# apache/yunikorn-k8shim

Measured on AMD Instinct MI355X. Metric: pod×node predicate evals/sec + decisions/sec, 50k nodes × 1M pods, higher is better.
Workload: dtype int64; 1 GPU; configs[2]: 50k nodes x 1M pods, NodeResourcesFit + TaintToleration + NodeAffinity; nodes_per_gpu=50000, total_nodes=50000, pods=1000000, templates=2000, pod_classes=2061, signature_planes=327, unique_requests=False, spread=False, gang_size=0, parallelism=single GPU

## Files before the change

yunikorn-k8shim_amd/csrc/engine/engine.hip:

```cpp
#include "../../../include/ykpred.h"

#include <hip/hip_runtime.h>
#include <dlfcn.h>
#include <rccl/rccl.h>

#include <algorithm>
#include <chrono>
#include <cstdio>
#include <cstdlib>
#include <cstring>
#include <mutex>
#include <string>
#include <unordered_map>
#include <vector>

#include "kernels.hip.h"

using ykk::i64;
using ykk::u64;

namespace {

thread_local std::string g_create_error;

// ... 187 lines not shown
  int64_t spread_cells = 0;
  bool spread_dirty = true;
  int res_vectors = 0;
  std::vector<i64> h_dim_val;
  std::vector<int32_t> h_dim_of;
  std::vector<int32_t> h_stage_rows;
  DevBuf d_dim_val, d_dim_order, d_dim_chunk_dim, d_dim_chunk_begin, d_dim_chunk_len, d_res_rows;
  int dim_chunks = 0;
  int walk_rows = 256;
  int wave_combine_below = 16;
  int n_big = 0, walk_chunks = 0, index_rows = 0;
  int NCB = 0;
  DevBuf d_big_dim, d_walk_big, d_walk_begin, d_walk_len, d_sfree_c, d_pmask_c, d_sfree_r, d_pmask_r, d_rbits_c;
  std::vector<int32_t> h_res_rows;
  std::vector<int32_t> h_row_pos;
  std::vector<int32_t> h_row_big;
  std::vector<int32_t> h_sorted_off;
  DevBuf d_sorted, d_sorted_off, d_ent_c;
  int sweep_min_run = 1;
  int sweep_groups = 0;
  bool sweep_ready = false;
  std::vector<int32_t> h_class_sweep;
  int sweep_rows[ykk::kMaxIdxRows] = {0, 0}, sweep_row_off[ykk::kMaxIdxRows + 1] = {0, 0, 0}, sweep_runs = 0;
  int index_rows_needed = 0;
  DevBuf d_agree;
  DevBuf d_explain;
  DevBuf d_headroom;
  DevBuf d_bytes_gather;
  DevBuf d_topo_agree;
  u64 dict_digest = 0;
  int fuse_rows = 1;
  int fuse_wpl = 0;
  int fuse_count = 0, fuse_row_count = 0;
  bool fuse_ready = false;
  DevBuf d_fuse_rec;
  int fuse_combos = 0;
  int fuse_combine = 1;
  DevBuf d_fuse_combo_rec, d_fuse_combo;
  std::vector<uint8_t> h_class_fused;
  int run_decide = 1;
  int run_ranges = 0, n_decide_list = 0, run_decide_classes = -1;
  bool win_partial = false;
  DevBuf d_run_ranges, d_no_decide, d_glin_r;
  int class_runs = 1;
  int class_runs_min_rows = 16;
  int run_classes = 0, run_units = 0, run_rows = 0;
  DevBuf d_run_classes, d_run_units;
  DevBuf d_sweep_rows, d_sweep_runs, d_sweep_units;
  int sweep_units[ykk::kMaxIdxRows] = {0, 0}, sweep_unit_off[ykk::kMaxIdxRows + 1] = {0, 0, 0};
  DevBuf d_chunk_list_b0;
  int NCB0 = 0;
  DevBuf d_walk2_order, d_walk2_big, d_walk2_begin, d_walk2_len;
  int walk2_chunks = -1;
  DevBuf d_first_r;
  static constexpr bool decide_skip = true;
  DevBuf d_chunk_list_b;
  DevBuf d_slice_general;
  DevBuf d_slice_desc;
  DevBuf d_pfx_r;
  DevBuf d_idx_c;
  DevBuf d_win_r;
  int idx_stride = 0;
  DevBuf d_sig_tol, d_sig_tolflags, d_sig_ports, d_swanted;
  DevBuf d_sig_aff_flags, d_sig_aff_off, d_sig_aff_terms, d_sig_pre_off, d_sig_pre_terms;
  bool specs_set = false;

  int P = 0, C = 0, NC = 0;
  std::vector<int32_t> h_pod_spec, h_pod_pin;
  DevBuf d_pod_spec, d_pod_pin, d_pod_class;
  DevBuf d_class_sig, d_class_pin, d_class_first, d_class_word, d_chunk_class, d_chunk_begin, d_chunk_len, d_chunk_first, d_members;
  std::unordered_map<ClassKey, int32_t, ClassKeyHash> class_ids;
  std::vector<int32_t> h_pod_class, h_pod_slot;
  std::vector<int32_t> h_pod_row;
  int rows_total = 0, rows_a = 0, row_capacity = 0;
  DevBuf d_pod_row;
  bool bands_enabled = true;
  int band_steps = 0;
  int band_steps_now = 128;
  int round_batched = -1;
  int round_node_assume = 1;
  int round_prof = 0;
  int fail_after = 0;
  int sig_wpl = 0;
  int combine_slices = 1;
  int decide_groups_from = 16384;
  int early_counts = 1;
  int max_lds_bytes = 64 * 1024;
  int num_cus = 256;
  int n_bands = 0, n_band_steps = 0, n_classes_a = 0, n_fix_rows = 0;
  std::vector<int32_t> h_class_slot_a;
  DevBuf d_band_tab, d_class_rows_a, d_class_list_a, d_class_slot_a, d_fix_row, d_fix_slot, d_chunk_zone;
  DevBuf d_class_list_b;
  int n_classes_b = 0;
  std::vector<int32_t> h_ch_zone;
  std::vector<uint8_t> h_row_stale;
  std::vector<int32_t> h_class_sig, h_class_pin, h_class_first, h_class_live;
  std::vector<std::vector<int32_t>> h_class_chunks;
  std::vector<int32_t> h_members, h_ch_class, h_ch_begin, h_ch_len, h_ch_first;
  int patch_chunks = 0;
  bool rank_valid = false;
  uint64_t specs_version = 1, ranked_specs_version = 0, ranked_nodes_epoch = 0;
  unsigned ranked_pre = 0, ranked_filt = 0;
  bool ranked_has_first = false;
  DevBuf d_round;
  DevBuf d_fx_off, d_fx_cls, d_fx_cnt, d_fx_occ, d_sp_sig_of;
  uint64_t fx_version = 0;
  bool fx_contrib = false, fx_ports = false;
  std::vector<int32_t> h_fx_off;
  std::vector<int32_t> h_fx_cls;
  std::vector<uint8_t> h_fx_occupies;
  DevBuf d_patches, d_rows, d_row_count, d_row_best;
  unsigned last_pre = 0, last_filt = 0;
  bool last_eval_valid = false;
  DevBuf d_class_count, d_class_best;
  bool pods_set = false, classes_dirty = true;
  int chunk_members = ykk::kChunkMembers;
  bool chunk_sorted = true;
  int combine_lds_bytes = 40000;

  DevBuf d_bitmap, d_counts, d_decisions, d_keys, d_scratch;
  void* last_bitmap = nullptr;
  int64_t last_bitmap_rows = 0;
  void *last_counts = nullptr, *last_decisions = nullptr, *last_keys = nullptr;

  hipStream_t aux_stream = nullptr;
  hipEvent_t ev_fork = nullptr, ev_planes = nullptr, ev_join = nullptr, ev_counts = nullptr, ev_zero = nullptr;
  hipStream_t peek_stream = nullptr;
  hipEvent_t ev_eval_done = nullptr;
  void* peek_pinned = nullptr;
  size_t peek_pinned_bytes = 0;

  struct GraphKey {
    uint64_t version;
    unsigned pre, filt, options;
    void *bitmap, *counts, *decisions, *keys;
    bool operator==(const GraphKey& o) const {
      return version == o.version && pre == o.pre && filt == o.filt && options == o.options && bitmap == o.bitmap && counts == o.counts &&
             decisions == o.decisions && keys == o.keys;
    }
  };
  std::vector<std::pair<GraphKey, hipGraphExec_t>> graphs;
  std::vector<GraphKey> seen;
  uint64_t tables_version = 1;
  bool graph_disabled = true;

  ncclComm_t comm = nullptr;
  int comm_rank = 0, comm_world = 1, node_offset = 0;
  int64_t round_exchanges = 0;
  void* h_round_pinned = nullptr;
  size_t h_round_pinned_bytes = 0;
  int64_t rounds_batched = 0, round_batched_asks = 0, round_batches = 0, rounds_sequential = 0, round_sequential_asks = 0;
  int forced_stride = 0;
  DevBuf d_gathered, d_gathered_map, d_xkey, d_xcand;
  bool last_has_keys = false;
  DevBuf d_class_rows_all, d_gathered_classes, d_class_rows_slot, d_class_sig_ident, d_expand_count, d_layout_hash, d_gathered_pod_class, d_row_pod;
  int ident_classes = 0;
  uint64_t layout_version = 1, layout_hashed_version = 0, layout_hash_value = 0, row_pod_version = 0;
  uint64_t ask_epoch = 1, hdr_epoch = 0;
  std::vector<uint64_t> hdr_cache;
  uint64_t nodes_epoch = 1, hist_epoch = 0;
  uint64_t bitmap_epoch = 0;

  int64_t n_full_evals = 0, n_node_patches = 0, n_row_patches = 0, n_queries = 0, n_gathers = 0, n_uploads = 0;

  hipEvent_t ev[2 * YKPRED_MAX_TIMED_KERNELS + 2]{};
  bool ev_ready = false;
// ... 1059 lines not shown

#define YK_SERIALISE(eng) \
  std::unique_lock<std::recursive_mutex> engine_lock; \
  if (eng) engine_lock = std::unique_lock<std::recursive_mutex>((eng)->mu)

extern "C" {

int32_t ykpred_abi_version(void) { return YKPRED_ABI_VERSION; }

const char* ykpred_last_error(const ykpred_engine_t* e) { return e ? e->err.c_str() : g_create_error.c_str(); }

int32_t ykpred_create(const ykpred_config_t* cfg, ykpred_engine_t** out) {
  if (!cfg || !out) {
    g_create_error = "null argument";
    return YKPRED_E_INVALID;
  }
  if (cfg->abi_version != YKPRED_ABI_VERSION) {
    g_create_error = "ABI version mismatch";
    return YKPRED_E_INVALID;
  }
  if (cfg->num_resources < 3 || cfg->num_resources > ykk::kMaxR || cfg->taint_words < 1 || cfg->taint_words > ykk::kMaxKT ||
      cfg->label_words < 1 || cfg->label_words > ykk::kMaxWTotal) {
    g_create_error = "config out of range: need 3<=R<=8, 1<=KT<=4, 1<=W<=32";
    return YKPRED_E_UNSUPPORTED;
  }
  if (cfg->topology_keys < 0 || cfg->topology_keys > ykk::kMaxKD || cfg->selector_classes < 0 || cfg->selector_classes > 4096 ||
      cfg->port_words < 0 || cfg->port_words > ykk::kMaxKP) {
    g_create_error = "config out of range: need 0<=KD<=8 topology keys, 0<=KS<=4096 selector classes, 0<=KP<=4 port words";
    return YKPRED_E_UNSUPPORTED;
  }
  int ndev = 0;
  hipError_t s = hipGetDeviceCount(&ndev);
  if (s != hipSuccess || ndev <= 0) {
    g_create_error = std::string("no HIP device: ") + hipGetErrorString(s) + " (libykpred has no CPU fallback)";
    return YKPRED_E_DEVICE;
  }
  if (cfg->device < 0 || cfg->device >= ndev) {
    g_create_error = "device ordinal out of range";
    return YKPRED_E_INVALID;
  }
  s = hipSetDevice(cfg->device);
  if (s != hipSuccess) {
    g_create_error = std::string("hipSetDevice: ") + hipGetErrorString(s);
    return YKPRED_E_DEVICE;
  }
  auto* e = new ykpred_engine();
  e->cfg = *cfg;
  e->R = cfg->num_resources;
  e->KT = cfg->taint_words;
  e->W = cfg->label_words;
  e->KD = cfg->topology_keys;
  e->KS = cfg->selector_classes;
  e->KP = cfg->port_words;
  if (cfg->reserved[0] >= 1 && cfg->reserved[0] <= ykk::kChunkMembers) e->chunk_members = cfg->reserved[0];
  e->chunk_sorted = cfg->reserved[1] != 1;
  if (cfg->reserved[2] > 0 && cfg->reserved[2] <= 160 * 1024) e->combine_lds_bytes = cfg->reserved[2];
  if (cfg->reserved[2] < 0) e->combine_lds_bytes = 0;
  if (cfg->reserved[4] > 0) e->walk_rows = cfg->reserved[4];
  if (cfg->reserved[5] > 0) e->wave_combine_below = cfg->reserved[5];
  if (cfg->reserved[5] < 0) e->wave_combine_below = 0;
  if (cfg->reserved[6] < 0) e->bands_enabled = false;
  if (cfg->reserved[6] > 0) e->band_steps = std::min(256, std::max(4, (cfg->reserved[6] + 3) / 4 * 4));
  e->graph_disabled = cfg->reserved[3] != 1;
  {
    int lds = 0;
    if (hipDeviceGetAttribute(&lds, hipDeviceAttributeMaxSharedMemoryPerBlock, cfg->device) == hipSuccess && lds > 0) e->max_lds_bytes = lds;
    int cus = 0;
    if (hipDeviceGetAttribute(&cus, hipDeviceAttributeMultiprocessorCount, cfg->device) == hipSuccess && cus > 0) e->num_cus = cus;
  }
  if (const char* tune = getenv("YKPRED_TUNE")) {
    std::string text(tune);
    size_t at = 0;
    while (at < text.size()) {
      size_t stop = text.find(',', at);
      if (stop == std::string::npos) stop = text.size();
      const std::string item = text.substr(at, stop - at);
      at = stop + 1;
      if (item.empty()) continue;
      const size_t eq = item.find('=');
      const std::string key = item.substr(0, eq);
      const int val = eq == std::string::npos ? 1 : atoi(item.c_str() + eq + 1);
      if (key == "walk_rows") e->walk_rows = std::max(val, 1);
      else if (key == "sig_wpl") e->sig_wpl = val;
      else if (key == "combine_slices") e->combine_slices = val;
      else if (key == "decide_groups_from") e->decide_groups_from = val;
      else if (key == "graph") e->graph_disabled = val != 1;
      else if (key == "early_counts") e->early_counts = val;
      else if (key == "band_steps") {
        e->bands_enabled = val >= 0;
        e->band_steps = val > 0 ? std::min(256, std::max(4, (val + 3) / 4 * 4)) : 0;
      } else if (key == "chunk_members") e->chunk_members = std::min(std::max(val, 1), (int)ykk::kChunkMembers);
      else if (key == "wave_combine_below") e->wave_combine_below = std::max(val, 0);
      else if (key == "fail_after") e->fail_after = std::max(val, 0);
      else if (key == "round_prof") e->round_prof = val;
      else if (key == "round_batched") e->round_batched = val;
      else if (key == "round_node_assume") e->round_node_assume = val;
      else if (key == "sweep_min_run") e->sweep_min_run = std::max(val, 0);
      else if (key == "sweep_groups") e->sweep_groups = std::max(val, 0);
      else if (key == "class_runs") e->class_runs = val;
      else if (key == "run_decide") e->run_decide = val;
      else if (key == "fuse_rows") e->fuse_rows = val;
      else if (key == "fuse_wpl") e->fuse_wpl = val;
      else if (key == "fuse_combine") e->fuse_combine = val;
      else if (key == "class_runs_min_rows") e->class_runs_min_rows = std::max(val, 1);
      else {
        g_create_error = "YKPRED_TUNE: unknown key '" + key + "'";
        delete e;
        return YKPRED_E_INVALID;
      }
    }
  }
  s = hipStreamCreateWithFlags(&e->own_stream, hipStreamNonBlocking);
  if (s != hipSuccess) {
    g_create_error = std::string("hipStreamCreate: ") + hipGetErrorString(s);
    delete e;
    return YKPRED_E_DEVICE;
  }
  {
    int lo = 0, hi = 0;
    (void)hipDeviceGetStreamPriorityRange(&lo, &hi);
    if (hipStreamCreateWithPriority(&e->aux_stream, hipStreamNonBlocking, hi) != hipSuccess)
      (void)hipStreamCreateWithFlags(&e->aux_stream, hipStreamNonBlocking);
  }
  if (hipStreamCreateWithFlags(&e->peek_stream, hipStreamNonBlocking) != hipSuccess) e->peek_stream = nullptr;
  (void)hipEventCreateWithFlags(&e->ev_eval_done, hipEventDisableTiming);
  (void)hipEventCreateWithFlags(&e->ev_fork, hipEventDisableTiming);
  (void)hipEventCreateWithFlags(&e->ev_join, hipEventDisableTiming);
  (void)hipEventCreateWithFlags(&e->ev_planes, hipEventDisableTiming);
  (void)hipEventCreateWithFlags(&e->ev_counts, hipEventDisableTiming);
  (void)hipEventCreateWithFlags(&e->ev_zero, hipEventDisableTiming);
  for (auto& ev : e->ev) (void)hipEventCreate(&ev);
  e->ev_ready = true;
  *out = e;
  return YKPRED_OK;
}

void ykpred_destroy(ykpred_engine_t* e) {
  if (!e) return;
  (void)hipSetDevice(e->cfg.device);
  (void)hipDeviceSynchronize();
  if (e->comm) (void)rccl()->CommDestroy(e->comm);
  e->comm = nullptr;
  for (DevBuf* b : {&e->d_gathered, &e->d_gathered_map, &e->d_xkey, &e->d_xcand}) b->release();
  for (auto& g : e->graphs) (void)hipGraphExecDestroy(g.second);
  e->graphs.clear();
  for (DevBuf* b : {&e->d_alloc, &e->d_req, &e->d_allowed, &e->d_count, &e->d_nflags, &e->d_taints, &e->d_labels, &e->d_domain, &e->d_selcount, &e->d_ports, &e->d_sig_ports, &e->d_swanted,
                    &e->d_sp_cnt_prev, &e->d_sp_present_prev, &e->d_sp_min_prev, &e->d_sig_changed, &e->d_class_dirty,
                    &e->d_spec_spread, &e->d_sp_coff, &e->d_sp_c, &e->d_sp_aff, &e->d_sp_tol, &e->d_sp_cnt, &e->d_sp_present, &e->d_sp_min,
                    &e->planes_canon, &e->planes_ranked, &e->base_canon, &e->base_ranked, &e->d_rankbuf, &e->d_score, &e->d_key,
                    &e->d_rank, &e->d_perm, &e->d_sreq, &e->d_stol, &e->d_sflags, &e->d_aff_off, &e->d_aff_terms, &e->d_pre_off,
                    &e->d_pre_terms, &e->d_dim_val, &e->d_dim_order, &e->d_dim_chunk_dim, &e->d_dim_chunk_begin, &e->d_dim_chunk_len,
                    &e->d_res_rows, &e->d_big_dim, &e->d_walk_big, &e->d_walk_begin, &e->d_walk_len, &e->d_sfree_c, &e->d_pmask_c,
                    &e->d_sfree_r, &e->d_pmask_r, &e->d_rbits_c, &e->d_sorted, &e->d_sorted_off, &e->d_ent_c, &e->d_agree, &e->d_topo_agree, &e->d_bytes_gather, &e->d_fuse_rec, &e->d_fuse_combo_rec, &e->d_fuse_combo, &e->d_run_ranges, &e->d_no_decide, &e->d_glin_r, &e->d_run_classes, &e->d_run_units, &e->d_sweep_rows, &e->d_sweep_runs, &e->d_sweep_units, &e->d_chunk_list_b0, &e->d_walk2_order, &e->d_walk2_big, &e->d_walk2_begin, &e->d_walk2_len, &e->d_idx_c, &e->d_win_r, &e->d_pfx_r, &e->d_slice_desc, &e->d_slice_general, &e->d_chunk_list_b, &e->d_first_r, &e->d_sig_tol, &e->d_sig_tolflags, &e->d_sig_aff_flags, &e->d_sig_aff_off,
                    &e->d_sig_aff_terms, &e->d_sig_pre_off, &e->d_sig_pre_terms, &e->d_pod_spec, &e->d_pod_pin, &e->d_pod_class,
                    &e->d_class_sig, &e->d_class_pin, &e->d_class_first, &e->d_class_word, &e->d_chunk_class, &e->d_chunk_begin, &e->d_chunk_len, &e->d_chunk_first,
                    &e->d_pod_row, &e->d_band_tab, &e->d_class_rows_a, &e->d_class_list_a, &e->d_class_slot_a, &e->d_fix_row, &e->d_fix_slot, &e->d_chunk_zone,
                    &e->d_members, &e->d_patches, &e->d_rows, &e->d_row_count, &e->d_row_best, &e->d_class_count, &e->d_class_best, &e->d_bitmap, &e->d_counts, &e->d_decisions, &e->d_keys, &e->d_scratch,
                    &e->d_member_key, &e->d_name_rank, &e->d_member_tie, &e->d_class_rows_all, &e->d_gathered_classes, &e->d_class_rows_slot,
                    &e->d_class_sig_ident, &e->d_expand_count, &e->d_layout_hash, &e->d_gathered_pod_class, &e->d_row_pod,
                    &e->d_round, &e->d_fx_off, &e->d_fx_cls, &e->d_fx_cnt, &e->d_fx_occ, &e->d_sp_sig_of, &e->d_class_list_b, &e->d_gathered, &e->d_gathered_map,
                    &e->d_xkey, &e->d_xcand})
    b->release();
  if (e->ev_ready)
    for (auto& ev : e->ev) (void)hipEventDestroy(ev);
  if (e->ev_fork) (void)hipEventDestroy(e->ev_fork);
  if (e->ev_join) (void)hipEventDestroy(e->ev_join);
// ... 592 lines not shown
                     use_run_decide ? e->d_no_decide.as<int>() : nullptr};
  ykk::Planes pc{res_on ? o_res.canon : nullptr, o_tol.canon, aff_on ? o_aff.canon : nullptr, spread_on ? o_spread.canon : nullptr,
                 e->row_stride, e->d_res_rows.as<int>(), 1 + e->R, e->d_idx_c.as<unsigned char>(), e->idx_stride, e->d_pmask_c.as<u64>(), e->row_words,
                 nullptr, 0, 0, 0, 0, 0, nullptr, nullptr, nullptr, nullptr, nullptr};
  int* first_r = nullptr;
  if ((a->options & (YKPRED_OUT_DECISIONS | YKPRED_OUT_DECISION_KEYS)) && e->decide_skip) {
    HIPCHK(e->d_first_r.ensure((size_t)std::max(e->plane_rows_alloc, 1) * sizeof(int)));
    first_r = e->d_first_r.as<int>();
  }
  if (want_dec && res_on && e->n_big > 0 && !fit_error) HIPCHK(e->d_pfx_r.ensure((size_t)e->n_big * (size_t)std::max(e->row_words, 1) * sizeof(i64)));
  ykk::Planes pr = ranked_planes_of(e, pre, filt, spread_on, first_r != nullptr);
  pc.n_big = pr.n_big;
  pc.rbits = e->d_rbits_c.as<u64>();
  const int pin_on = ((filt & YKPRED_PLUGIN_NODE_NAME) ? 1 : 0) | (spread_err ? 2 : 0);
  hipStream_t sb = e->aux_stream;

  if (want_dec) {
    HIPCHK(hipEventRecord(e->ev_fork, st));
    HIPCHK(hipStreamWaitEvent(sb, e->ev_fork, 0));
    if (zero_counts_beside) {
      HIPCHK(hipMemsetAsync(e->d_class_count.p, 0, (size_t)e->C * sizeof(int), sb));
      HIPCHK(hipEventRecord(e->ev_zero, sb));
    }
    if (first_r) HIPCHK(hipMemsetAsync(first_r, 0x7f, (size_t)std::max(e->plane_rows_alloc, 1) * sizeof(int), sb));
    tm.begin(sb);
    hipLaunchKernelGGL(ykk::k_score, dim3((unsigned)nblk_nodes), dim3(ykk::kBlock), 0, sb, nt, e->d_score.as<double>(), e->d_key.as<u64>());
    tm.end(sb, "k_score");
    int* hist = e->d_rankbuf.as<int>();
    int* bucket_off = hist + ykk::kRankBuckets;
    int* cursor = bucket_off + ykk::kRankBuckets + 1;
    int* members = cursor + ykk::kRankBuckets;
    HIPCHK(hipMemsetAsync(hist, 0, ykk::kRankBuckets * sizeof(int), sb));
    tm.begin(sb);
    hipLaunchKernelGGL(ykk::k_rank_hist, dim3((unsigned)nblk_nodes), dim3(ykk::kBlock), 0, sb, N, e->d_score.as<double>(), hist);
    hipLaunchKernelGGL(ykk::k_rank_scan, dim3(1), dim3(ykk::kRankBuckets), 0, sb, hist, bucket_off, cursor);
    hipLaunchKernelGGL(ykk::k_rank_fill, dim3((unsigned)nblk_nodes), dim3(ykk::kBlock), 0, sb, N, e->d_score.as<double>(), e->d_key.as<u64>(),
                       e->has_name_rank ? e->d_name_rank.as<int>() : (const int*)nullptr, cursor, members, e->d_member_tie.as<int>(),
                       e->d_member_key.as<u64>());
    hipLaunchKernelGGL(ykk::k_rank_final, dim3((unsigned)ykk::kRankBuckets), dim3(ykk::kBlock), 0, sb, bucket_off, members,
                       e->d_member_tie.as<int>(), e->d_member_key.as<u64>(), e->d_rank.as<int>(), e->d_perm.as<int>());
    tm.end(sb, "k_rank");
  }
  auto base_of = [&](DevBuf& buf) {
    ykk::BasePlanes bp;
    bp.req = buf.as<u64>();
    bp.taint = bp.req + (size_t)64 * e->W * e->row_stride;
    bp.port = bp.taint + (size_t)64 * e->KT * e->row_stride;
    bp.unsched = bp.port + (size_t)64 * e->KP * e->row_stride;
    bp.exists = bp.unsched + e->row_stride;
    bp.stride = e->row_stride;
    return bp;
  };
  auto launch_dictionary_planes = [&](hipStream_t s, const int* perm, bool ranked, const char* base_name, const char* sig_name, bool base_done = false) -> int {
    ykk::BasePlanes bp = base_of(ranked ? e->base_ranked : e->base_canon);
    if (!base_done) {
      tm.begin(s);
      hipLaunchKernelGGL(ykk::k_base_planes, dim3((unsigned)(e->W + e->KT + e->KP + 1), wgroups), dim3(ykk::kBlock), 0, s, nt, perm, bp,
                         e->row_words);
      tm.end(s, base_name);
    }
    ykk::SigPlaneArgs sa{};
    sa.base = bp;
    sa.tol = o_tol;
    sa.aff = o_aff;
    if (ranked) {
      sa.tol.canon = o_tol.ranked;
      sa.aff.canon = o_aff.ranked;
      sa.tol.first = first_r ? first_r + e->fam_tol.base : nullptr;
      sa.aff.first = first_r ? first_r + e->fam_aff.base : nullptr;
    }
    if (!aff_on) sa.aff.D = 0;
    sa.sig_tol = e->d_sig_tol.as<u64>();
    sa.sig_tolflags = e->d_sig_tolflags.as<unsigned>();
    sa.sig_ports = e->d_sig_ports.as<u64>();
    sa.KP = e->KP;
    for (int k = 0; k < ykk::kMaxKT; ++k) sa.taint_used[k] = e->taint_used[k];
    sa.affs = as;
    sa.KT = e->KT;
    sa.W = e->W;
    sa.pre_mask = pre;
    sa.filt_mask = filt;
    sa.n_words = e->row_words;
    tm.begin(s);
    const int wpl = e->sig_wpl > 0 ? e->sig_wpl : (e->row_words >= 4 * ykk::kWave ? 4 : (e->row_words >= 2 * ykk::kWave ? 2 : 1));
    const unsigned chunks = std::max((unsigned)((std::max(sa.tol.D, sa.aff.D) + ykk::kBitSigsPerBlock - 1) / ykk::kBitSigsPerBlock), 1u);
    const unsigned ygroups = (unsigned)((e->row_words + ykk::kBlock * wpl - 1) / (ykk::kBlock * wpl));
    if (wpl >= 4)
      hipLaunchKernelGGL(ykk::k_sig_planes<4>, dim3(chunks, ygroups, 2u), dim3(ykk::kBlock), 0, s, sa);
    else if (wpl >= 2)
      hipLaunchKernelGGL(ykk::k_sig_planes<2>, dim3(chunks, ygroups, 2u), dim3(ykk::kBlock), 0, s, sa);
    else
      hipLaunchKernelGGL(ykk::k_sig_planes<1>, dim3(chunks, ygroups, 2u), dim3(ykk::kBlock), 0, s, sa);
    tm.end(s, sig_name);
    return YKPRED_OK;
  };
  if (want_dec) TRY(launch_dictionary_planes(sb, e->d_perm.as<int>(), true, "k_base_planes(ranked)", "k_sig_planes(ranked)"));
  auto ranked_walk = [](const int* perm) { return perm != nullptr; };
  auto launch_ballot_planes = [&](hipStream_t s, const int* perm, const char* name, bool with_base = false) {
    ykk::PlaneArgs pa{};
    pa.perm = perm;
    pa.res = o_res;
    pa.spread = o_spread;
    if (perm && first_r) {
      pa.res.first = first_r + e->fam_res.base;
      pa.spread.first = first_r + e->fam_spread.base;
    }
    if (!spread_on) pa.spread.D = 0;
    pa.dims = ykk::DimPlanes{e->d_dim_val.as<i64>(), e->d_dim_order.as<int>(), e->d_dim_chunk_dim.as<int>(), e->d_dim_chunk_begin.as<int>(),
                             e->d_dim_chunk_len.as<int>(), res_on ? e->dim_chunks : 0};
    pa.spreads = spread_sigs(e);
    pa.fit_error = fit_error;
    pa.n_words = e->row_words;
    pa.spread_en = pts_en ? 1 : 0;
    pa.ipa_en = ipa_en ? 1 : 0;
    unsigned xchunks = std::max((unsigned)pa.dims.n_chunks, sig_chunks(pa.spread.D));
    tm.begin(s);
    if (with_base) {
      xchunks = std::max(xchunks, (unsigned)(e->W + e->KT + e->KP + 1));
      hipLaunchKernelGGL(ykk::k_node_planes, dim3(std::max(xchunks, 1u), wgroups, 3u), dim3(ykk::kBlock), 0, s, nt, pa,
                         base_of(perm ? e->base_ranked : e->base_canon));
    } else {
      hipLaunchKernelGGL(ykk::k_planes, dim3(std::max(xchunks, 1u), wgroups, spread_on ? 2u : 1u), dim3(ykk::kBlock), 0, s, nt, pa);
    }
    tm.end(s, name);
    if (res_on && e->n_big > 0 && !fit_error) {
      const bool ranked = perm != nullptr;
      ykk::DimWalk dw{e->d_dim_val.as<i64>(), e->d_dim_order.as<int>(), e->d_big_dim.as<int>(), e->d_walk_big.as<int>(), e->d_walk_begin.as<int>(),
                      e->d_walk_len.as<int>(), (ranked ? e->d_sfree_r : e->d_sfree_c).as<i64>(), (ranked ? e->d_pmask_r : e->d_pmask_c).as<u64>(),
                      e->n_big, e->walk_chunks, e->row_words, ranked ? nullptr : e->d_rbits_c.as<u64>(),
                      (!ranked && sweep_rows_on) ? e->d_ent_c.as<unsigned>() : nullptr, e->d_sorted.as<i64>(), e->d_sorted_off.as<int>(),
                      (ranked && use_run_decide) ? e->d_glin_r.as<unsigned>() : nullptr};
      tm.begin(s);
      hipLaunchKernelGGL(ykk::k_dim_sort, dim3((unsigned)e->n_big, wgroups), dim3(ykk::kBlock), 0, s, nt, perm, dw);
      tm.end(s, ranked ? "k_dim_sort(ranked)" : "k_dim_sort");
      tm.begin(s);
      const unsigned walk_gy = (unsigned)((e->row_words + ykk::kBlock * ykk::kWalkWords - 1) / (ykk::kBlock * ykk::kWalkWords));
      const dim3 walk_grid((unsigned)e->walk_chunks, walk_gy);
      if (!ranked && use_sweep && e->walk2_chunks >= 0) {
        if (e->walk2_chunks > 0) {
          ykk::DimWalk dw2 = dw;
          dw2.order = e->d_walk2_order.as<int>();
          dw2.chunk_big = e->d_walk2_big.as<int>();
          dw2.chunk_begin = e->d_walk2_begin.as<int>();
          dw2.chunk_len = e->d_walk2_len.as<int>();
          dw2.n_chunks = e->walk2_chunks;
          hipLaunchKernelGGL(ykk::k_dim_walk, dim3((unsigned)e->walk2_chunks, walk_gy), dim3(ykk::kBlock), 0, s, dw2, e->d_idx_c.as<unsigned char>(), e->idx_stride);
        }
      } else if (!ranked) {
        hipLaunchKernelGGL(ykk::k_dim_walk, walk_grid, dim3(ykk::kBlock), 0, s, dw, e->d_idx_c.as<unsigned char>(), e->idx_stride);
      } else {
        hipLaunchKernelGGL(ykk::k_dim_prefix_max, dim3((unsigned)e->n_big), dim3(ykk::kPfxBlock), 0, s, dw, e->d_pfx_r.as<i64>());
        if (use_run_decide) {
          if (e->walk2_chunks > 0) {
            ykk::DimWalk dw2 = dw;
            dw2.order = e->d_walk2_order.as<int>();
            dw2.chunk_big = e->d_walk2_big.as<int>();
            dw2.chunk_begin = e->d_walk2_begin.as<int>();
            dw2.chunk_len = e->d_walk2_len.as<int>();
            dw2.n_chunks = e->walk2_chunks;
            hipLaunchKernelGGL(ykk::k_dim_walk_window<8>, dim3((unsigned)e->walk2_chunks, walk_gy), dim3(ykk::kBlock), 0, s, dw2, e->d_pfx_r.as<i64>(), e->d_win_r.as<unsigned char>());
          }
        } else {
          hipLaunchKernelGGL(ykk::k_dim_walk_window<ykk::kWalkBatch>, walk_grid, dim3(ykk::kBlock), 0, s, dw, e->d_pfx_r.as<i64>(), e->d_win_r.as<unsigned char>());
        }
      }
      tm.end(s, ranked ? "k_dim_walk(ranked)" : "k_dim_walk");
    } else if (res_on && e->n_big > 0) {
      if (!ranked_walk(perm)) (void)hipMemsetAsync(e->d_idx_c.p, 64, (size_t)e->fam_res.D * (size_t)e->idx_stride, s);
      (void)hipMemsetAsync((ranked_walk(perm) ? e->d_pmask_r : e->d_pmask_c).p, 0, (size_t)e->n_big * (size_t)e->row_words * 65 * sizeof(u64), s);
      if (!ranked_walk(perm)) (void)hipMemsetAsync(e->d_rbits_c.p, 0, (size_t)e->n_big * (size_t)e->row_words * ykk::kRankBits * sizeof(u64), s);
    }
  };
  const bool fused_planes = res_on || spread_on;
  if (fused_planes) launch_ballot_planes(st, nullptr, "k_planes+k_base_planes", true);
  TRY(launch_dictionary_planes(st, nullptr, false, "k_base_planes", "k_sig_planes", fused_planes));
// ... 159 lines not shown
      const unsigned ygroups = (unsigned)((e->row_words + gw - 1) / gw);
      ykk::FuseSrc fsrc{e->planes_canon.as<u64>(), e->fuse_combos > 0 ? e->d_fuse_combo.as<u64>() : nullptr, {e->fam_res.base, e->fam_tol.base, e->fam_aff.base}};
      tm.begin(sz);
      auto launch_fused = [&](auto kernel, const ykk::FuseRec* recs, int n, u64* out, int* counts) {
        hipLaunchKernelGGL(kernel, dim3((unsigned)((n + ykk::kFuseRecsPerBlock - 1) / ykk::kFuseRecsPerBlock), ygroups), dim3(ykk::kBlock), 0, sz, recs, n, fsrc,
                           e->row_words, e->row_stride, out, counts);
      };
      auto launch_wide = [&](const ykk::FuseRec* recs, int n, u64* out, int* counts) {
        if (wpl == 5) launch_fused(ykk::k_fused_rows<5, 8>, recs, n, out, counts);
        else if (wpl == 2) launch_fused(ykk::k_fused_rows<2, 8>, recs, n, out, counts);
        else launch_fused(ykk::k_fused_rows<1, 8>, recs, n, out, counts);
      };
      if (e->fuse_combos > 0) {
        launch_wide(e->d_fuse_combo_rec.as<ykk::FuseRec>(), e->fuse_combos, e->d_fuse_combo.as<u64>(), nullptr);
        if (wpl == 5) launch_fused(ykk::k_fused_rows<5, 2>, e->d_fuse_rec.as<ykk::FuseRec>(), e->fuse_count, bitmap, e->d_class_count.as<int>());
        else if (wpl == 2) launch_fused(ykk::k_fused_rows<2, 2>, e->d_fuse_rec.as<ykk::FuseRec>(), e->fuse_count, bitmap, e->d_class_count.as<int>());
        else launch_fused(ykk::k_fused_rows<1, 2>, e->d_fuse_rec.as<ykk::FuseRec>(), e->fuse_count, bitmap, e->d_class_count.as<int>());
      } else {
        launch_wide(e->d_fuse_rec.as<ykk::FuseRec>(), e->fuse_count, bitmap, e->d_class_count.as<int>());
      }
      tm.end(sz, "k_fused_rows");
    }
    tm.begin(sz);
    int walk_nit = 0, walk_segs = 0, walk_long = 0;
    ykk::WalkStage wstage{};
    wstage.n = (int)e->h_stage_rows.size();
    for (int k = 0; k < wstage.n; ++k) wstage.row[k] = e->h_stage_rows[(size_t)k];
    bool slices = small_chunks && e->combine_slices != 0 && pc.n_big > 0 && pc.res != nullptr && !(use_sweep && e->sweep_min_run <= 1 && listed);
    if (slices) {
      const int its = (e->row_stride + ykk::kWave - 1) / ykk::kWave;
      const size_t lds_cap = std::min((size_t)e->max_lds_bytes, (size_t)80 * 1024);
      walk_segs = (its + ykk::kWalkMaxIt - 1) / ykk::kWalkMaxIt;
      walk_nit = (its + walk_segs - 1) / walk_segs;
      while (walk_nit > 1 && ykk::walk_lds_bytes(pc.n_big, wstage.n, walk_nit) > lds_cap) {
        ++walk_segs;
        walk_nit = (its + walk_segs - 1) / walk_segs;
      }
      walk_long = walk_segs - (walk_nit * walk_segs - its);
      slices = ykk::walk_lds_bytes(pc.n_big, wstage.n, walk_nit) <= (size_t)e->max_lds_bytes && its * ykk::kWave <= e->idx_stride;
    }
    if (slices) {
      HIPCHK(e->d_slice_desc.ensure((size_t)std::max(e->NC, 1) * sizeof(ykk::SliceDesc)));
      HIPCHK(e->d_slice_general.ensure(sizeof(int)));
      HIPCHK(hipMemsetAsync(e->d_slice_general.p, 0, sizeof(int), sz));
      hipLaunchKernelGGL(ykk::k_slice_desc, dim3((unsigned)((e->NC + ykk::kBlock - 1) / ykk::kBlock)), dim3(ykk::kBlock), 0, sz, ct, pc, e->NC, class_dirty,
                         pin_on, e->d_slice_desc.as<ykk::SliceDesc>(), e->d_slice_general.as<int>(), wstage);
      tm.end(sz, "k_slice_desc");
      tm.begin(sz);
      const int per_group = ykk::kRowsWaves * ykk::kWalkChunksPerWave;
      const unsigned gx = (unsigned)((e->NC + per_group - 1) / per_group);
      auto launch_walk = [&](auto kernel, int nit, int segs, int w_base) -> int {
        const size_t lds = ykk::walk_lds_bytes(pc.n_big, wstage.n, nit);
        if (lds > 64 * 1024) HIPCHK(hipFuncSetAttribute((const void*)kernel, hipFuncAttributeMaxDynamicSharedMemorySize, (int)lds));
        hipLaunchKernelGGL(kernel, dim3(gx, (unsigned)segs), dim3(ykk::kRowsThreads), lds, sz, pc, e->d_slice_desc.as<ykk::SliceDesc>(), bitmap,
                           e->row_words, e->row_stride, pin_on, e->d_class_count.as<int>(), e->NC, w_base, wstage);
        return YKPRED_OK;
      };
      auto launch_segments = [&](int nit, int segs, int w_base, bool tail) -> int {
        if (segs <= 0) return YKPRED_OK;
        switch (nit * 2 + (tail ? 1 : 0)) {
#define YK_WALK_CASE(N)                                                         \
  case (N) * 2: return launch_walk(ykk::k_walk_rows<(N), false>, nit, segs, w_base); \
  case (N) * 2 + 1: return launch_walk(ykk::k_walk_rows<(N), true>, nit, segs, w_base);
          YK_WALK_CASE(1) YK_WALK_CASE(2) YK_WALK_CASE(3) YK_WALK_CASE(4) YK_WALK_CASE(5) YK_WALK_CASE(6) YK_WALK_CASE(7)
#undef YK_WALK_CASE
        }
        return fail(e, YKPRED_E_INVALID, "k_walk_rows: no kernel for " + std::to_string(nit) + " word groups per lane");
      };
      {
        const int n_short = walk_segs - walk_long, nit_last = n_short > 0 ? walk_nit - 1 : walk_nit;
        const int long_plain = n_short > 0 ? walk_long : walk_long - 1, short_plain = n_short > 0 ? n_short - 1 : 0;
        TRY(launch_segments(walk_nit, long_plain, 0, false));
        TRY(launch_segments(walk_nit - 1, short_plain, walk_long * walk_nit * ykk::kWave, false));
        TRY(launch_segments(nit_last, 1, (long_plain * walk_nit + short_plain * (walk_nit - 1)) * ykk::kWave, true));
      }
      tm.end(sz, "k_walk_rows");
      tm.begin(sz);
      hipLaunchKernelGGL(ykk::k_combine_wave, dim3((unsigned)((e->NC + ykk::kWavesPerBlock - 1) / ykk::kWavesPerBlock)), dim3(ykk::kBlock), 0, sz, ct,
                         pc, bitmap, e->row_words, e->row_stride, pin_on, e->d_class_count.as<int>(), e->NC, class_dirty,
                         e->d_slice_desc.as<ykk::SliceDesc>(), e->d_slice_general.as<int>(), (const int*)nullptr);
    } else if (counts_early) {
      const ykk::FixRows fix{e->d_class_rows_a.as<u64>(), e->d_fix_row.as<int>(), e->d_fix_slot.as<int>(), e->n_fix_rows};
      const int blocks = n_run + e->n_fix_rows;
      if (blocks > 0)
        hipLaunchKernelGGL(ykk::k_combine, dim3((unsigned)blocks, grid.y), dim3(ykk::kBlock), (size_t)e->combine_lds_bytes, sz, ct, pc, bitmap, e->row_words,
                           e->row_stride, pin_on, (int*)nullptr, tpg, class_dirty, chunk_list, fix, n_run);
    } else if (n_run == 0) {
    } else if (small_chunks) {
      const dim3 wgrid((unsigned)((std::max(n_run, 1) + ykk::kWavesPerBlock - 1) / ykk::kWavesPerBlock));
      hipLaunchKernelGGL(ykk::k_combine_wave, wgrid, dim3(ykk::kBlock), 0, sz, ct, pc, bitmap, e->row_words, e->row_stride, pin_on,
                         e->d_class_count.as<int>(), n_run, class_dirty, (const ykk::SliceDesc*)nullptr, (const int*)nullptr, chunk_list);
    } else {
      hipLaunchKernelGGL(ykk::k_combine, grid, dim3(ykk::kBlock), (size_t)e->combine_lds_bytes, sz, ct, pc, bitmap, e->row_words, e->row_stride,
                         pin_on, e->d_class_count.as<int>(), tpg, class_dirty, chunk_list, ykk::FixRows{nullptr, nullptr, nullptr, 0}, n_run);
    }
    tm.end(sz, dirty_only ? "k_combine(dirty classes)" : "k_combine");
  }
  if (want_dec) {
    HIPCHK(hipEventRecord(e->ev_join, sb));
    HIPCHK(hipStreamWaitEvent(st, e->ev_join, 0));
  }
  if ((want_dec || want_cnt) && !scattered) {
    tm.begin(st);
    hipLaunchKernelGGL(ykk::k_scatter, dim3((unsigned)((P + ykk::kBlock - 1) / ykk::kBlock)), dim3(ykk::kBlock), 0, st, P,
                       e->d_pod_class.as<int>(), e->d_class_count.as<int>(), e->d_class_best.as<int>(), e->d_key.as<u64>(),
                       want_cnt ? (int*)e->last_counts : nullptr, want_dec ? (int*)e->last_decisions : nullptr,
                       want_keys ? (i64*)e->last_keys : nullptr);
    tm.end(st, "k_scatter");
  }
  HIPCHK(hipGetLastError());
  return YKPRED_OK;
  };
  const bool graphable = !tm.on && !e->graph_disabled && !(e->comm && e->comm_world > 1) && !(a->options & (YKPRED_EVAL_DIRECT | YKPRED_EVAL_SPREAD_COUNT_ONLY));
  hipGraphExec_t exec = nullptr;
  if (graphable) {
    ykpred_engine::GraphKey key{e->tables_version, pre, filt, a->options, (void*)bitmap, e->last_counts, e->last_decisions, e->last_keys};
    for (size_t i = 0; i < e->graphs.size();) {
      if (e->graphs[i].first.version != e->tables_version) {
        (void)hipGraphExecDestroy(e->graphs[i].second);
        e->graphs.erase(e->graphs.begin() + (long)i);
      } else {
        if (e->graphs[i].first == key) exec = e->graphs[i].second;
        ++i;
      }
    }
    bool repeated = false;
    for (size_t i = 0; i < e->seen.size();) {
      if (e->seen[i].version != e->tables_version) {
        e->seen.erase(e->seen.begin() + (long)i);
        continue;
      }
      repeated = repeated || e->seen[i] == key;
      ++i;
    }
    if (!repeated && e->seen.size() < 8) e->seen.push_back(key);
    if (!exec && repeated) {
      hipGraph_t g = nullptr;
      int crc = YKPRED_E_DEVICE;
      if (hipStreamBeginCapture(st, hipStreamCaptureModeThreadLocal) == hipSuccess) {
        crc = enqueue();
        if (hipStreamEndCapture(st, &g) != hipSuccess) crc = YKPRED_E_DEVICE;
      }
      if (crc == YKPRED_OK && g && hipGraphInstantiate(&exec, g, nullptr, nullptr, 0) == hipSuccess) {
        if (e->graphs.size() >= 8) {
          (void)hipGraphExecDestroy(e->graphs.front().second);
          e->graphs.erase(e->graphs.begin());
        }
        e->graphs.emplace_back(key, exec);
      } else {
        exec = nullptr;
        e->graph_disabled = true;
        (void)hipGetLastError();
      }
      if (g) (void)hipGraphDestroy(g);
    }
  }
  if (exec) {
    HIPCHK(hipGraphLaunch(exec, st));
  } else {
    int rc = enqueue();
    if (rc < 0) return rc;
    if (rc == 1) {
      tm.done(st);
      return YKPRED_OK;
    }
  }
// ... 2079 lines not shown
```

yunikorn-k8shim_amd/csrc/engine/kernels.hip.h:

```cpp
#pragma once
#include <hip/hip_runtime.h>
#include <stdint.h>

#include <type_traits>

namespace ykk {

typedef unsigned long long u64;
typedef long long i64;

constexpr int kMaxR = 8;
constexpr int kMaxKT = 4;
constexpr int kMaxW = 8;
constexpr int kMaxWTotal = 32;
constexpr int kMaxKD = 8;
constexpr int kMaxKP = 4;

constexpr int kWave = 64;
constexpr int kBlock = 256;
constexpr int kWavesPerBlock = kBlock / kWave;
constexpr int kSigsPerBlock = 16;
constexpr int kSigsPerBlockMany = 64;
constexpr int kManySigs = 4096;
__host__ __device__ inline int sigs_per_block(int D) { return D > kManySigs ? kSigsPerBlockMany : kSigsPerBlock; }
// ... 488 lines not shown
    }
    u64* dst = is_label ? o.req + (size_t)(c * 64 + lane) * o.stride
                        : (is_taint ? o.taint + (size_t)((c - t.W) * 64 + lane) * o.stride
                                    : o.port + (size_t)((c - t.W - t.KT) * 64 + lane) * o.stride);
    dst[word] = keep;
  } else {
    u64 un = __ballot(n >= 0 && (t.flags[n >= 0 ? n : 0] & kNodeUnschedulable));
    u64 ex = __ballot(n >= 0);
    if (lane == 0) {
      o.unsched[word] = un;
      o.exists[word] = ex;
    }
  }
}

__global__ __launch_bounds__(kBlock) void k_base_planes(NodeTable t, const int* __restrict__ perm, BasePlanes o, int n_words) {
  if ((int)blockIdx.x < t.W + t.KT + t.KP + 1) plane_base(t, perm, o, n_words);
}

struct SigPlaneArgs {
  BasePlanes base;
  PlaneOut tol, aff;
  const u64* sig_tol;
  const unsigned* sig_tolflags;
  const u64* sig_ports;
  int KP;
  u64 taint_used[kMaxKT];
  AffSigs affs;
  int KT, W;
  unsigned pre_mask, filt_mask;
  int n_words;
};
constexpr int kBitSigsPerBlock = 8;

template <int WPL>
__device__ __forceinline__ void dnf_words(const u64* __restrict__ terms, int t0, int t1, int W, const u64* __restrict__ req, int stride,
                                          const int (&w)[WPL], u64 (&any)[WPL]) {
#pragma unroll
  for (int j = 0; j < WPL; ++j) any[j] = 0;
  for (int t = t0; t < t1; ++t) {
    u64 all[WPL];
#pragma unroll
    for (int j = 0; j < WPL; ++j) all[j] = ~0ull;
    for (int k = 0; k < W; ++k) {
      u64 m = terms[(size_t)t * W + k];
      while (m) {
        int q = __ffsll((long long)m) - 1;
        m &= m - 1;
        const u64* row = req + (size_t)(k * 64 + q) * stride;
#pragma unroll
        for (int j = 0; j < WPL; ++j) all[j] &= row[w[j]];
      }
    }
#pragma unroll
    for (int j = 0; j < WPL; ++j) any[j] |= all[j];
  }
}
constexpr int kSigTermRegs = 4;
template <int WPL>
__device__ __forceinline__ void dnf_words_regs(const u64 (&tw)[kSigTermRegs], int j0, int j1, int W, const u64* __restrict__ req, int stride,
                                               const int (&w)[WPL], u64 (&any)[WPL]) {
#pragma unroll
  for (int j = 0; j < WPL; ++j) any[j] = 0;
  for (int jj = j0; jj < j1;) {
    u64 all[WPL];
#pragma unroll
    for (int j = 0; j < WPL; ++j) all[j] = ~0ull;
    for (int k = 0; k < W; ++k, ++jj) {
      const int r = jj >> 6, l = jj & 63;
      u64 m = (u64)readlane_i64((i64)(r == 0 ? tw[0] : (r == 1 ? tw[1] : (r == 2 ? tw[2] : tw[3]))), l);
      while (m) {
        int q = __ffsll((long long)m) - 1;
        m &= m - 1;
        const u64* row = req + (size_t)(k * 64 + q) * stride;
#pragma unroll
        for (int j = 0; j < WPL; ++j) all[j] &= row[w[j]];
      }
    }
#pragma unroll
    for (int j = 0; j < WPL; ++j) any[j] |= all[j];
  }
}
template <int WPL>
__global__ __launch_bounds__(kBlock) void k_sig_planes(SigPlaneArgs a) {
  const int lane = threadIdx.x % kWave;
  const int wbase = (blockIdx.y * kWavesPerBlock + threadIdx.x / kWave) * (kWave * WPL);
  if (wbase >= a.n_words) return;
  int w[WPL], w_raw[WPL];
  bool live[WPL];
  u64 exists[WPL];
#pragma unroll
  for (int j = 0; j < WPL; ++j) {
    w_raw[j] = wbase + j * kWave + lane;
    live[j] = w_raw[j] < a.n_words;
    w[j] = live[j] ? w_raw[j] : a.n_words - 1;
    exists[j] = a.base.exists[w[j]];
  }
  auto note_first = [&](int* first, int d, const u64 (&val)[WPL]) {
    if (!first) return;
    int fw = kNoWord;
#pragma unroll
    for (int j = WPL - 1; j >= 0; --j) {
      const u64 nz = __ballot(live[j] && val[j] != 0);
      if (nz) fw = wbase + j * kWave + __ffsll((long long)nz) - 1;
    }
    if (fw != kNoWord && lane == 0) atomicMin(&first[d], fw);
  };
  const int d0 = blockIdx.x * kBitSigsPerBlock;
  if (blockIdx.z == 0) {
    const int nd = min(kBitSigsPerBlock, a.tol.D - d0);
    if (nd <= 0) return;
    const bool taint_en = a.filt_mask & kPlugTaint, unsched_en = a.filt_mask & kPlugUnsched;
    const bool ports_en = (a.filt_mask & kPlugPorts) && (a.pre_mask & kPlugPorts);
    u64 unsched[WPL];
#pragma unroll
    for (int j = 0; j < WPL; ++j) unsched[j] = unsched_en ? a.base.unsched[w[j]] : 0ull;
    const bool batch = nd * a.KT <= kWave && nd * a.KP <= kWave;
    const unsigned fl_l = lane < nd ? a.sig_tolflags[d0 + lane] : 0u;
    u64 tol_l = 0, port_l = 0;
    if (batch) {
      if (lane < nd * a.KT) tol_l = a.sig_tol[(size_t)d0 * a.KT + lane];
      if (ports_en && lane < nd * a.KP) port_l = a.sig_ports[(size_t)d0 * a.KP + lane];
    }
    for (int i = 0; i < nd; ++i) {
      const int d = d0 + i;
      const unsigned fl = (unsigned)__builtin_amdgcn_readlane((int)fl_l, i);
      u64 bad[WPL];
#pragma unroll
      for (int j = 0; j < WPL; ++j) bad[j] = 0;
      if (taint_en)
        for (int k = 0; k < a.KT; ++k) {
          const u64 tolerated = batch ? (u64)readlane_i64((i64)tol_l, i * a.KT + k) : a.sig_tol[(size_t)d * a.KT + k];
          u64 m = ~tolerated & a.taint_used[k];
          while (m) {
            int tt = __ffsll((long long)m) - 1;
            m &= m - 1;
            const u64* row = a.base.taint + (size_t)(k * 64 + tt) * a.base.stride;
#pragma unroll
            for (int j = 0; j < WPL; ++j) bad[j] |= row[w[j]];
          }
        }
      if (ports_en)
        for (int k = 0; k < a.KP; ++k) {
          u64 m = batch ? (u64)readlane_i64((i64)port_l, i * a.KP + k) : a.sig_ports[(size_t)d * a.KP + k];
          while (m) {
            int pp = __ffsll((long long)m) - 1;
            m &= m - 1;
            const u64* row = a.base.port + (size_t)(k * 64 + pp) * a.base.stride;
#pragma unroll
            for (int j = 0; j < WPL; ++j) bad[j] |= row[w[j]];
          }
        }
      u64 val[WPL];
#pragma unroll
      for (int j = 0; j < WPL; ++j) {
        u64 b = bad[j];
        if (!(fl & kSpecToleratesUnsched)) b |= unsched[j];
        if (fl & kSpecUnsupported) b = ~0ull;
        val[j] = exists[j] & ~b;
        if (live[j]) a.tol.canon[(size_t)d * a.tol.stride + w[j]] = val[j];
      }
      note_first(a.tol.first, d, val);
    }
  } else {
    const int nd = min(kBitSigsPerBlock, a.aff.D - d0);
    if (nd <= 0) return;
    const bool pre_en = a.pre_mask & kPlugAffinity, filt_en = a.filt_mask & kPlugAffinity;
    const unsigned f_l = lane < nd ? a.affs.flags[d0 + lane] : 0u;
    const int to_l = lane <= nd ? a.affs.term_off[d0 + lane] : 0;
    const int tbase = __builtin_amdgcn_readlane(to_l, 0);
    const int n_mask_words = (__builtin_amdgcn_readlane(to_l, nd) - tbase) * a.W;
    const bool batch = filt_en && n_mask_words <= kSigTermRegs * kWave;
    u64 tw[kSigTermRegs];
#pragma unroll
    for (int r = 0; r < kSigTermRegs; ++r) {
      const int j = r * kWave + lane;
      tw[r] = batch && j < n_mask_words ? a.affs.terms[(size_t)tbase * a.W + j] : 0ull;
    }
    for (int i = 0; i < nd; ++i) {
      const int d = d0 + i;
      const unsigned f = (unsigned)__builtin_amdgcn_readlane((int)f_l, i);
      const bool skip = pre_en && (f & kSpecAffSkip);
      u64 ok[WPL];
#pragma unroll
      for (int j = 0; j < WPL; ++j) ok[j] = exists[j];
      if (pre_en && !skip) {
        if (f & kSpecPreReject) {
#pragma unroll
          for (int j = 0; j < WPL; ++j) ok[j] = 0;
        }
        if (f & kSpecPreNames) {
          u64 any[WPL];
          dnf_words<WPL>(a.affs.pre_terms, a.affs.pre_off[d], a.affs.pre_off[d + 1], a.W, a.base.req, a.base.stride, w, any);
#pragma unroll
          for (int j = 0; j < WPL; ++j) ok[j] &= any[j];
        }
      }
      if (filt_en && !skip) {
        const int t0 = __builtin_amdgcn_readlane(to_l, i), t1 = __builtin_amdgcn_readlane(to_l, i + 1);
        u64 any[WPL];
        if (batch)
          dnf_words_regs<WPL>(tw, (t0 - tbase) * a.W, (t1 - tbase) * a.W, a.W, a.base.req, a.base.stride, w, any);
        else
          dnf_words<WPL>(a.affs.terms, t0, t1, a.W, a.base.req, a.base.stride, w, any);
#pragma unroll
        for (int j = 0; j < WPL; ++j) ok[j] &= any[j];
      }
#pragma unroll
      for (int j = 0; j < WPL; ++j)
        if (live[j]) a.aff.canon[(size_t)d * a.aff.stride + w[j]] = ok[j];
      note_first(a.aff.first, d, ok);
    }
  }
}

__global__ __launch_bounds__(kBlock) void k_permute_planes(int n_nodes, const int* __restrict__ perm, const u64* __restrict__ canon,
                                                           u64* __restrict__ ranked, int stride, int n_rows, int n_words,
                                                           int* __restrict__ first ) {
  const int wave = threadIdx.x / kWave, lane = threadIdx.x % kWave;
  const int w = blockIdx.y * kWavesPerBlock + wave;
  if (w >= n_words) return;
  const int pos = w * kWave + lane;
  const int src = pos < n_nodes ? perm[pos] : -1;
  const int sw = src >> 6, sb = src & 63;
  const int spb = sigs_per_block(n_rows);
  const int d0 = blockIdx.x * spb;
  const int dend = min(d0 + spb, n_rows);
  u64 keep = 0;
  for (int d = d0; d < dend; ++d) {
    bool bit = src >= 0 && ((canon[(size_t)d * stride + sw] >> sb) & 1ull);
    u64 b = __ballot(bit);
    if (d - d0 == lane) keep = b;
  }
  if (lane < dend - d0) {
    ranked[(size_t)(d0 + lane) * stride + w] = keep;
    if (first && keep) atomicMin(&first[d0 + lane], w);
  }
}

struct SpreadC {
  int kd, ks, max_skew, min_domains, self_match;
  unsigned flags;
  int cnt_off, dom_size;
  int kind;
};
struct SpreadSigs {
  int D;
  const int* c_off;
// ... 3346 lines not shown
```

Before: 40800 billion evals/s.

## Adapt signature-plane grid to fill CUs and run combine tail on side stream

Makes signatures-per-block a runtime parameter of k_sig_planes and, by default, halves signatures-per-block and then words-per-lane until the grid has about four blocks per CU, so small signature/word counts still occupy the GPU. Separately, when classes are scattered and no sweep/fuse path is active, it launches the early k_combine on the secondary stream so it can overlap with other work. This trades more blocks and less per-block reuse of the loaded taint/term data for parallelism, and adds cross-stream ordering risk.

```diff
diff --git a/yunikorn-k8shim_amd/csrc/engine/engine.hip b/yunikorn-k8shim_amd/csrc/engine/engine.hip
--- a/yunikorn-k8shim_amd/csrc/engine/engine.hip
+++ b/yunikorn-k8shim_amd/csrc/engine/engine.hip
@@ -293,6 +293,8 @@
   int round_prof = 0;
   int fail_after = 0;
   int sig_wpl = 0;
+  int sig_per_block = 0;
+  int tail_beside = 1;
   int combine_slices = 1;
   int decide_groups_from = 16384;
   int early_counts = 1;
@@ -1518,6 +1520,8 @@
       const int val = eq == std::string::npos ? 1 : atoi(item.c_str() + eq + 1);
       if (key == "walk_rows") e->walk_rows = std::max(val, 1);
       else if (key == "sig_wpl") e->sig_wpl = val;
+      else if (key == "sig_per_block") e->sig_per_block = val;
+      else if (key == "tail_beside") e->tail_beside = val;
       else if (key == "combine_slices") e->combine_slices = val;
       else if (key == "decide_groups_from") e->decide_groups_from = val;
       else if (key == "graph") e->graph_disabled = val != 1;
@@ -2276,15 +2280,25 @@
     sa.filt_mask = filt;
     sa.n_words = e->row_words;
     tm.begin(s);
-    const int wpl = e->sig_wpl > 0 ? e->sig_wpl : (e->row_words >= 4 * ykk::kWave ? 4 : (e->row_words >= 2 * ykk::kWave ? 2 : 1));
-    const unsigned chunks = std::max((unsigned)((std::max(sa.tol.D, sa.aff.D) + ykk::kBitSigsPerBlock - 1) / ykk::kBitSigsPerBlock), 1u);
+    int wpl = e->sig_wpl > 0 ? (e->sig_wpl >= 4 ? 4 : (e->sig_wpl >= 2 ? 2 : 1)) : (e->row_words >= 4 * ykk::kWave ? 4 : (e->row_words >= 2 * ykk::kWave ? 2 : 1));
+    int spb = e->sig_per_block > 0 ? (e->sig_per_block >= 8 ? 8 : (e->sig_per_block >= 4 ? 4 : (e->sig_per_block >= 2 ? 2 : 1))) : ykk::kBitSigsPerBlock;
+    const int sigs = std::max(std::max(sa.tol.D, sa.aff.D), 1);
+    auto sig_blocks = [&](int per_block, int words_per_lane) {
+      return (long)((sigs + per_block - 1) / per_block) * ((e->row_words + ykk::kBlock * words_per_lane - 1) / (ykk::kBlock * words_per_lane)) * 2;
+    };
+    const long want_blocks = 4L * e->num_cus;
+    if (e->sig_per_block <= 0)
+      while (spb > 1 && sig_blocks(spb, wpl) < want_blocks) spb /= 2;
+    if (e->sig_wpl <= 0)
+      while (wpl > 1 && sig_blocks(spb, wpl) < want_blocks) wpl /= 2;
+    const unsigned chunks = (unsigned)((sigs + spb - 1) / spb);
     const unsigned ygroups = (unsigned)((e->row_words + ykk::kBlock * wpl - 1) / (ykk::kBlock * wpl));
     if (wpl >= 4)
-      hipLaunchKernelGGL(ykk::k_sig_planes<4>, dim3(chunks, ygroups, 2u), dim3(ykk::kBlock), 0, s, sa);
+      hipLaunchKernelGGL(ykk::k_sig_planes<4>, dim3(chunks, ygroups, 2u), dim3(ykk::kBlock), 0, s, sa, spb);
     else if (wpl >= 2)
-      hipLaunchKernelGGL(ykk::k_sig_planes<2>, dim3(chunks, ygroups, 2u), dim3(ykk::kBlock), 0, s, sa);
+      hipLaunchKernelGGL(ykk::k_sig_planes<2>, dim3(chunks, ygroups, 2u), dim3(ykk::kBlock), 0, s, sa, spb);
     else
-      hipLaunchKernelGGL(ykk::k_sig_planes<1>, dim3(chunks, ygroups, 2u), dim3(ykk::kBlock), 0, s, sa);
+      hipLaunchKernelGGL(ykk::k_sig_planes<1>, dim3(chunks, ygroups, 2u), dim3(ykk::kBlock), 0, s, sa, spb);
     tm.end(s, sig_name);
     return YKPRED_OK;
   };
@@ -2610,6 +2624,10 @@
     } else if (counts_early) {
       const ykk::FixRows fix{e->d_class_rows_a.as<u64>(), e->d_fix_row.as<int>(), e->d_fix_slot.as<int>(), e->n_fix_rows};
       const int blocks = n_run + e->n_fix_rows;
+      if (scattered && e->tail_beside != 0 && !(use_sweep && e->run_classes > 0) && !sweep_rows_on && !fuse_on) {
+        sz = sb;
+        tm.begin(sz);
+      }
       if (blocks > 0)
         hipLaunchKernelGGL(ykk::k_combine, dim3((unsigned)blocks, grid.y), dim3(ykk::kBlock), (size_t)e->combine_lds_bytes, sz, ct, pc, bitmap, e->row_words,
                            e->row_stride, pin_on, (int*)nullptr, tpg, class_dirty, chunk_list, fix, n_run);
diff --git a/yunikorn-k8shim_amd/csrc/engine/kernels.hip.h b/yunikorn-k8shim_amd/csrc/engine/kernels.hip.h
--- a/yunikorn-k8shim_amd/csrc/engine/kernels.hip.h
+++ b/yunikorn-k8shim_amd/csrc/engine/kernels.hip.h
@@ -594,7 +594,7 @@
   }
 }
 template <int WPL>
-__global__ __launch_bounds__(kBlock) void k_sig_planes(SigPlaneArgs a) {
+__global__ __launch_bounds__(kBlock) void k_sig_planes(SigPlaneArgs a, int spb) {
   const int lane = threadIdx.x % kWave;
   const int wbase = (blockIdx.y * kWavesPerBlock + threadIdx.x / kWave) * (kWave * WPL);
   if (wbase >= a.n_words) return;
@@ -618,9 +618,9 @@
     }
     if (fw != kNoWord && lane == 0) atomicMin(&first[d], fw);
   };
-  const int d0 = blockIdx.x * kBitSigsPerBlock;
+  const int d0 = blockIdx.x * spb;
   if (blockIdx.z == 0) {
-    const int nd = min(kBitSigsPerBlock, a.tol.D - d0);
+    const int nd = min(spb, a.tol.D - d0);
     if (nd <= 0) return;
     const bool taint_en = a.filt_mask & kPlugTaint, unsched_en = a.filt_mask & kPlugUnsched;
     const bool ports_en = (a.filt_mask & kPlugPorts) && (a.pre_mask & kPlugPorts);
@@ -675,7 +675,7 @@
       note_first(a.tol.first, d, val);
     }
   } else {
-    const int nd = min(kBitSigsPerBlock, a.aff.D - d0);
+    const int nd = min(spb, a.aff.D - d0);
     if (nd <= 0) return;
     const bool pre_en = a.pre_mask & kPlugAffinity, filt_en = a.filt_mask & kPlugAffinity;
     const unsigned f_l = lane < nd ? a.affs.flags[d0 + lane] : 0u;
```

Result: faster. 41810 billion evals/s, median of 6 (+2.5%).
